# skeskinen/bert.cpp

Measured on AMD Instinct MI355X. Metric: sentences/sec (seq_len=128), higher is better.
Workload: dtype f16; 1 GPU; all-MiniLM-L6-v2 f16, batch=256 seq_len=128; per_gpu_batch=256, global_batch=256, seq_len=128, weights=f16, parallelism=dp1 (replicated weights, sharded sentences)

## Files before the change

bert.cpp_amd/csrc/device.h:

```cpp
#pragma once
#include "kernels.h"

#include <cstdio>
#include <type_traits>
#include <utility>

namespace bert_hip {

typedef _Float16 f16x2 __attribute__((ext_vector_type(2)));
typedef _Float16 f16x4 __attribute__((ext_vector_type(4)));
typedef _Float16 f16x8 __attribute__((ext_vector_type(8)));
typedef float f32x2 __attribute__((ext_vector_type(2)));
typedef float f32x4 __attribute__((ext_vector_type(4)));
typedef float f32x8 __attribute__((ext_vector_type(8)));
typedef float f32x16 __attribute__((ext_vector_type(16)));
typedef uint32_t u32x4 __attribute__((ext_vector_type(4)));
typedef uint32_t u32x16 __attribute__((ext_vector_type(16)));
typedef int32_t i32x4 __attribute__((ext_vector_type(4)));
typedef int32_t i32x16 __attribute__((ext_vector_type(16)));

template <int... I, class F>
__device__ __forceinline__ void static_for_impl(std::integer_sequence<int, I...>, F &&f) {
    (f(std::integral_constant<int, I>{}), ...);
}
// ... 26 lines not shown
    }                                                                                                         \
} while (0)
#define TL_DUMP_RAW(cond, nstamps) do {                                                                      \
    static int tl_shots = 0;                                                                                  \
    if ((cond) && tl_shots++ == 20) {                                                                         \
        (void)hipDeviceSynchronize();                                                                         \
        static unsigned long long tl_h[1024 * 256];                                                           \
        (void)hipMemcpyFromSymbol(tl_h, HIP_SYMBOL(g_timeline), sizeof(tl_h));                                \
        for (int b : {0, 100}) {                                                                              \
            fprintf(stderr, "rawtimeline wg %3d:", b);                                                        \
            for (int i = 0; i < (nstamps); ++i)                                                               \
                fprintf(stderr, " %lld", tl_h[b * 256 + i] ? (long long)(tl_h[b * 256 + i] - tl_h[b * 256]) : -1LL); \
            fprintf(stderr, "\n");                                                                            \
        }                                                                                                     \
    }                                                                                                         \
} while (0)
#else
#define TL_DUMP_RAW(cond, nstamps) do { } while (0)
#define TL_REALTIME_AT(sel, i) do { } while (0)
#define TL_STAMP(i) do { } while (0)
#define TL_STAMP_AT(sel, i) do { } while (0)
#define TL_DUMP(cond, nstamps) do { } while (0)
#endif

__device__ __forceinline__ unsigned lds_addr(const void *p) {
    return (unsigned)(size_t)(__attribute__((address_space(3))) const char *)p;
}
template <bool MEMORY, int OFF, class V = f16x8>
__device__ __forceinline__ V lds_read_b128(unsigned addr) {
    static_assert(sizeof(V) == 16, "ds_read_b128 reads 16 bytes");
    static_assert(OFF >= 0 && OFF < 65536, "ds offset field is 16 bits");
    V v;
    if constexpr (MEMORY) asm volatile("ds_read_b128 %0, %1 offset:%2" : "=v"(v) : "v"(addr), "n"(OFF) : "memory");
    else asm volatile("ds_read_b128 %0, %1 offset:%2" : "=v"(v) : "v"(addr), "n"(OFF));
    return v;
}
template <class V>
__device__ __forceinline__ void landed(V &v) { asm volatile("" : "+v"(v)); }
template <int VM>
__device__ __forceinline__ void dma_barrier() {
    asm volatile("s_waitcnt vmcnt(%0) lgkmcnt(0)\n\ts_barrier" : : "n"(VM) : "memory");
}

__device__ __forceinline__ int off64(int row, int chunk) { return row * 128 + ((chunk ^ ((row >> 1) & 7)) << 4); }

__device__ __forceinline__ float rounded_f32(float v) {
    asm("" : "+v"(v));
    return v;
}

__device__ __forceinline__ void xor32_pair(float &a, float &b) {
    asm("s_nop 1\n\tv_permlane32_swap_b32 %0, %1\n\ts_nop 1" : "+v"(a), "+v"(b));
}
__device__ __forceinline__ float xor32_sum(float v) { float a = v, b = v; xor32_pair(a, b); return a + b; }
__device__ __forceinline__ float xor32_max(float v) { float a = v, b = v; xor32_pair(a, b); return __builtin_fmaxf(a, b); }
__device__ __forceinline__ float wave_sum_f32(float v) {
    v = xor32_sum(v);
    v += __builtin_bit_cast(float, __builtin_amdgcn_ds_swizzle(__builtin_bit_cast(int, v), (16 << 10) | 0x1F));
    v += __builtin_bit_cast(float, __builtin_amdgcn_ds_swizzle(__builtin_bit_cast(int, v), (8 << 10) | 0x1F));
    v += __builtin_bit_cast(float, __builtin_amdgcn_ds_swizzle(__builtin_bit_cast(int, v), (4 << 10) | 0x1F));
    v += __builtin_bit_cast(float, __builtin_amdgcn_mov_dpp(__builtin_bit_cast(int, v), 0x4E, 0xF, 0xF, true));
    v += __builtin_bit_cast(float, __builtin_amdgcn_mov_dpp(__builtin_bit_cast(int, v), 0xB1, 0xF, 0xF, true));
    return v;
}

#ifndef BERT_HIP_EXP16
#define BERT_HIP_EXP16 0
#endif
#if BERT_HIP_EXP16
typedef u32x4 sm_arg_t;
typedef u32x4 sm_exp_t;
__device__ __forceinline__ sm_arg_t softmax_args4(float s0, float s1, float s2, float s3, float s4, float s5, float s6, float s7, float sc, float m) {
    uint32_t a0, a1, a2, a3;
    asm("v_fma_mixlo_f16 %0, %4, %12, -%13\n\t"
        "v_fma_mixlo_f16 %1, %6, %12, -%13\n\t"
        "v_fma_mixlo_f16 %2, %8, %12, -%13\n\t"
        "v_fma_mixlo_f16 %3, %10, %12, -%13\n\t"
        "v_fma_mixhi_f16 %0, %5, %12, -%13\n\t"
        "v_fma_mixhi_f16 %1, %7, %12, -%13\n\t"
        "v_fma_mixhi_f16 %2, %9, %12, -%13\n\t"
        "v_fma_mixhi_f16 %3, %11, %12, -%13"
        : "=&v"(a0), "=&v"(a1), "=&v"(a2), "=&v"(a3)
        : "v"(s0), "v"(s1), "v"(s2), "v"(s3), "v"(s4), "v"(s5), "v"(s6), "v"(s7), "s"(sc), "v"(m));
    return u32x4{a0, a1, a2, a3};
}
__device__ __forceinline__ sm_exp_t softmax_exp4(sm_arg_t a) {
    uint32_t p0, p1, p2, p3;
    asm("v_exp_f16_e32 %0, %4\n\t"
        "v_exp_f16_e32 %1, %5\n\t"
        "v_exp_f16_e32 %2, %6\n\t"
        "v_exp_f16_e32 %3, %7\n\t"
        "v_exp_f16_sdwa %0, %4 dst_sel:WORD_1 dst_unused:UNUSED_PRESERVE src0_sel:WORD_1\n\t"
        "v_exp_f16_sdwa %1, %5 dst_sel:WORD_1 dst_unused:UNUSED_PRESERVE src0_sel:WORD_1\n\t"
        "v_exp_f16_sdwa %2, %6 dst_sel:WORD_1 dst_unused:UNUSED_PRESERVE src0_sel:WORD_1\n\t"
        "v_exp_f16_sdwa %3, %7 dst_sel:WORD_1 dst_unused:UNUSED_PRESERVE src0_sel:WORD_1\n\t"
        "s_nop 0"
        : "=&v"(p0), "=&v"(p1), "=&v"(p2), "=&v"(p3)
        : "v"(a[0]), "v"(a[1]), "v"(a[2]), "v"(a[3]));
    return u32x4{p0, p1, p2, p3};
}
__device__ __forceinline__ void softmax_sum4(sm_exp_t p, float &psum) {
    const f16x2 one = {(_Float16)1.0f, (_Float16)1.0f};
#pragma unroll
    for (int e = 0; e < 4; ++e) {
        const uint32_t pe = p[e];
        psum = __builtin_amdgcn_fdot2(__builtin_bit_cast(f16x2, pe), one, psum, false);
// ... 194 lines not shown
```

bert.cpp_amd/csrc/layer_tail.hip:

```cpp
#include "device.h"

namespace bert_hip {

namespace {

constexpr int LT_TILE = 16384;
#ifndef LT_ABLATE
#define LT_ABLATE 0
#endif
#ifndef LT_UPRIO
#define LT_UPRIO 1
#endif
#ifndef LT_GELU_BATCH
#define LT_GELU_BATCH 0
#endif
#ifndef LT_DMA_SPLIT
#define LT_DMA_SPLIT 1
#endif
#ifndef LT_DPRIO
#define LT_DPRIO 0
#endif

#ifdef BERT_HIP_TIMELINE
static __device__ unsigned long long g_tl_tail[256 * 512];
// ... 5 lines not shown
#endif
#else
#define LT_STAMP_FINE(sel, i) do { } while (0)
#define LT_STAMP(sel, i) do { } while (0)
#endif

struct TailArgs {
    const half_t *ctx, *x;
    const half_t *wo;
    const half_t *w1p;
    const half_t *w2p;
    const uint4 *wo_qs, *w1_qs, *w2_qs;
    const void *wo_sc, *w1_sc, *w2_sc;
    const float *bo, *g1, *be1, *b1, *b2, *g2, *be2;
    half_t *out;
    int I;
};

template <int N>
__device__ __forceinline__ void wait_frags(f16x8 (&f)[4]) {
    asm volatile("s_waitcnt lgkmcnt(%4)" : "+v"(f[0]), "+v"(f[1]), "+v"(f[2]), "+v"(f[3]) : "n"(N) : "memory");
}
template <int N>
__device__ __forceinline__ void wait_lgkm() {
    asm volatile("s_waitcnt lgkmcnt(%0)" : : "n"(N) : "memory");
}
template <int VM>
__device__ __forceinline__ void close_interval(f16x8 (&f)[4]) {
    asm volatile("s_waitcnt vmcnt(%4) lgkmcnt(0)\n\ts_barrier" : "+v"(f[0]), "+v"(f[1]), "+v"(f[2]), "+v"(f[3]) : "n"(VM) : "memory");
}
template <int OFF>
__device__ __forceinline__ f16x8 frag_read(unsigned addr) {
    if (LT_ABLATE & 4) { f16x8 z = (f16x8)(_Float16)0.f; asm volatile("" : "+v"(z) : "v"(addr)); return z; }
    return lds_read_b128<true, OFF>(addr);
}

__device__ __forceinline__ void dma_m0(unsigned lds) {
    if (LT_ABLATE & 1) return;
    asm volatile("s_mov_b32 m0, %0" : : "s"(lds) : "memory");
}
template <int PIECE>
__device__ __forceinline__ void dma_piece(const char *gbase, unsigned voff) {
    if (LT_ABLATE & 1) return;
    asm volatile("global_load_lds_dwordx4 %0, %1 offset:%2" : : "v"(voff), "s"(gbase - PIECE * 1024), "n"(PIECE * 1024) : "memory");
}

__device__ __forceinline__ f32x16 mfma16(const f16x8 &a, const f16x8 &b, const f32x16 &c) {
    if (LT_ABLATE & 8) { f32x16 r = c; asm volatile("" : "+v"(r[0]) : "v"(a), "v"(b)); return r; }
    return __builtin_amdgcn_mfma_f32_32x32x16_f16(a, b, c, 0, 0, 0);
}

}

template <int NT, int WT, bool RAGGED = false>
__device__ __forceinline__ void layer_tail_body(const TailArgs &a, char *smem, const int tok0, const int rows, const int tid) {
    constexpr bool Q4 = WT != GW_F16;
    constexpr int VMQ = Q4 ? 63 : 0;
    constexpr int H = 128 * NT, NBH = 2 * NT, NB = 4 * NT, NQ = 8 * NT, NYH = 4 * NT;
    constexpr int P = NT * NT;
    constexpr int NG = NT;
    constexpr int LAGT = NT + NG;
    const int I = a.I, NC = I / 64;
    const int lane = tid & 63;
    const int wave = __builtin_amdgcn_readfirstlane(tid >> 6);
    const int t = wave & 3, role = wave >> 2;
    const int l31 = lane & 31, hi = lane >> 5;
    const int tok_w = tok0 + t * 32;
    const int row_l = RAGGED ? tok0 + min(t * 32 + l31, rows - 1) : tok_w + l31;

    char *ringU = smem;
    char *ringD = smem + 3 * LT_TILE;
    char *G = smem + 6 * LT_TILE;
    float *ST = (float *)(G + 32768);
    float *cbo = ST + 8 * 64;
    float *cg1 = cbo + H, *cbe1 = cg1 + H, *cb2 = cbe1 + H, *cg2 = cb2 + H, *cbe2 = cg2 + H, *cb1 = cbe2 + H;

    {
        constexpr int NPB = 4;
        const float *const src[6] = {a.bo, a.g1, a.be1, a.b2, a.g2, a.be2};
        float pv[6];
        f32x4 bq[NPB];
#pragma unroll
        for (int k = 0; k < 6; ++k) pv[k] = tid < H ? src[k][tid] : 0.f;
#pragma unroll
        for (int k = 0; k < NPB; ++k) {
            const int i4 = (k * 512 + tid) * 4;
            bq[k] = i4 < I ? *(const f32x4 *)(a.b1 + i4) : f32x4{0.f, 0.f, 0.f, 0.f};
        }
        if (tid < H) {
#pragma unroll
            for (int k = 0; k < 6; ++k) cbo[k * H + tid] = pv[k];
        }
#pragma unroll
        for (int k = 0; k < NPB; ++k) {
            const int i4 = (k * 512 + tid) * 4;
            if (i4 < I + 128) *(f32x4 *)(cb1 + i4) = bq[k];
        }
    }
    f32x16 accp[NBH];
    f16x4 xv[NBH][4];
    {
        const half_t *xr = a.x + (size_t)row_l * H + role * 64 + 4 * hi;
#pragma unroll
        for (int b = 0; b < NBH; ++b)
#pragma unroll
            for (int gq = 0; gq < 4; ++gq) xv[b][gq] = *(const f16x4 *)(xr + (b >> 1) * 128 + (b & 1) * 32 + 8 * gq);
    }
    f16x8 bf[NQ];
// ... 356 lines not shown
                wait_frags<4>(Fb);
                LT_STAMP_FINE(fine, fb0 + 5);
                mm(Fb, I1{});
                LT_STAMP_FINE(fine, fb0 + 6);
                rd(3, Fc);
                wait_frags<4>(Fa);
                LT_STAMP_FINE(fine, fb0 + 7);
                mm(Fa, I2{});
                LT_STAMP_FINE(fine, fb0 + 8);
            } else {
                wait_lgkm<0>();
                bias_landed();
                static_for<12>([&](auto s_tag) __attribute__((always_inline)) { fill(std::integral_constant<int, 4 + decltype(s_tag)::value>{}); });
            }
            static_assert(MAXF <= 2, "two GELU batches per interval at most");
            pre_close();
            if constexpr (MMA) close_interval<VMQ>(Fc); else dma_barrier<VMQ>();
            next_slot();
        };
        using TT = std::true_type; using FF = std::false_type;
        LT_STAMP(tlU, 393);
        __builtin_amdgcn_s_setprio(LT_UPRIO);
        auto u_chunk = [&](auto par_tag, auto first_tag, int c) __attribute__((always_inline)) {
            constexpr bool FIRST = decltype(first_tag)::value;
            static_for<NT>([&](auto j_tag) __attribute__((always_inline)) {
                constexpr int j = decltype(j_tag)::value;
                constexpr bool carry = !(FIRST && j == 0), gelu = !FIRST && j < NG;
                u_interval(par_tag, j_tag, TT{}, std::integral_constant<bool, gelu>{}, std::integral_constant<bool, carry>{}, c);
            });
        };
        u_chunk(std::integral_constant<int, 0>{}, TT{}, 0);
        for (int c = 1; c + 1 < NC; c += 2) {
            u_chunk(std::integral_constant<int, 1>{}, FF{}, c);
            u_chunk(std::integral_constant<int, 0>{}, FF{}, c + 1);
        }
        u_chunk(std::integral_constant<int, 1>{}, FF{}, NC - 1);
        static_for<LAGT>([&](auto k_tag) __attribute__((always_inline)) {
            constexpr int k = decltype(k_tag)::value;
            if constexpr (k < NG)
                u_interval(std::integral_constant<int, 0>{}, std::integral_constant<int, k>{}, FF{}, TT{}, std::integral_constant<bool, k == 0>{}, NC);
            else {
                if constexpr (k == NG) {
                    char *const xu = ringU + t * (NYH * 1024) + lane * 16;
#pragma unroll
                    for (int m = 0; m < NYH; ++m) *(f16x8 *)(xu + m * 1024) = Y[8 * (m >> 2) + (m & 3)];
                }
                pre_close(); dma_barrier<VMQ>(); next_slot();
            }
        });
        static_assert(LAGT > NG, "U needs an idle interval to hand its half of y over");
        asm volatile("s_barrier" ::: "memory");
        asm volatile("s_barrier" ::: "memory");
        store_rows();
        return;
    } else {
        f16x8 yh[NYH];
        static_for<NBH>([&](auto b_tag) __attribute__((always_inline)) {
            constexpr int b = decltype(b_tag)::value;
            normalise_block(b_tag, yh[2 * b], yh[2 * b + 1]);
            *(f16x8 *)(xch + (2 * b) * 1024) = yh[2 * b];
            *(f16x8 *)(xch + (2 * b + 1) * 1024) = yh[2 * b + 1];
        });
        LT_STAMP(tlD, 400);
        asm volatile("s_waitcnt lgkmcnt(0)\n\ts_barrier" ::: "memory");
        f32x16 acc2[NB];
        static_for<NBH>([&](auto b_tag) __attribute__((always_inline)) {
            constexpr int b = decltype(b_tag)::value, n3 = b >> 1, obp = b & 1;
            f32x4 bu[4], bd[4];
#pragma unroll
            for (int gq = 0; gq < 4; ++gq) {
                bu[gq] = *(const f32x4 *)(cb2 + n3 * 128 + obp * 32 + 8 * gq + 4 * hi);
                bd[gq] = *(const f32x4 *)(cb2 + n3 * 128 + 64 + obp * 32 + 8 * gq + 4 * hi);
            }
#pragma unroll
            for (int gq = 0; gq < 4; ++gq)
#pragma unroll
                for (int e = 0; e < 4; ++e) {
                    acc2[4 * n3 + obp][4 * gq + e] = bu[gq][e];
                    acc2[4 * n3 + 2 + obp][4 * gq + e] = (float)yh[2 * b + (gq >> 1)][4 * (gq & 1) + e] + bd[gq][e];
                }
            asm volatile("" ::: "memory");
        });
        __builtin_amdgcn_s_waitcnt(0xc07f);
        const unsigned aD = aR + 3 * LT_TILE;
        const unsigned offI = rows_offset(I);
        auto dma_down = [&](int c, int n3, unsigned tile) __attribute__((always_inline)) {
            if constexpr (Q4) q4_request_rows(a.w2_qs, a.w2_sc, n3 * (I / 64) + c);
            else dma128(w2p + (size_t)n3 * 128 * I + c * 64, offI, I * 2, tile);
        };
        const unsigned aG = lds_addr(G) + (unsigned)(t * 8192 + lane * 16);
        const unsigned offU = up_offset();
        const int NUP = NC * NT;
        auto request = [&](auto up_tag, auto down_tag, int iu, int id) __attribute__((always_inline)) {
            const int s2 = slot_plus2();
            if constexpr (decltype(up_tag)::value) dma_up(iu / NT, iu % NT, offU, ldsU + s2 * LT_TILE);
            if constexpr (decltype(down_tag)::value) dma_down(id / NT, id % NT, ldsD + s2 * LT_TILE);
        };
        using TT = std::true_type; using FF = std::false_type;
        if (LT_DPRIO) __builtin_amdgcn_s_setprio(LT_DPRIO);
        static_for<LAGT>([&](auto k_tag) __attribute__((always_inline)) {
            constexpr int k = decltype(k_tag)::value;
            constexpr bool dn = k >= LAGT - 2;
            if constexpr (k >= 1) q4_expand_up(ringU + slot_plus1() * LT_TILE);
            if constexpr (k == LAGT - 1) q4_expand_rows(PERMUTED{}, ringD + slot_plus1() * LT_TILE);
            request(TT{}, std::integral_constant<bool, dn>{}, k + 2, k - (LAGT - 2));
            pre_close();
// ... 57 lines not shown
            });
        };
        static_assert(LAGT == 2 * NT, "the request schedule below assumes D runs two chunks behind");
        (void)NUP;
        for (int c = 0; c + 3 < NC; ++c) d_chunk(std::integral_constant<int, NT>{}, FF{}, TT{}, c);
        d_chunk(std::integral_constant<int, NT - 2>{}, FF{}, TT{}, NC - 3);
        d_chunk(std::integral_constant<int, 0>{}, FF{}, FF{}, NC - 2);
        d_chunk(std::integral_constant<int, 0>{}, TT{}, FF{}, NC - 1);

        {
            char *S = smem + t * (64 * H);
            int lane = (int)__builtin_amdgcn_mbcnt_hi(~0u, __builtin_amdgcn_mbcnt_lo(~0u, 0u));
            asm volatile("" : "+v"(lane));
            const int hi = lane >> 5;
            {
                const char *const xu = ringU + t * (NYH * 1024) + lane * 16;
#pragma unroll
                for (int n3 = 0; n3 < NT; ++n3) {
                    f16x8 yu[4];
#pragma unroll
                    for (int m = 0; m < 4; ++m) yu[m] = *(const f16x8 *)(xu + (4 * n3 + m) * 1024);
#pragma unroll
                    for (int m = 0; m < 4; ++m)
#pragma unroll
                        for (int e = 0; e < 8; ++e) acc2[4 * n3 + (m >> 1)][8 * (m & 1) + e] += (float)yu[m][e];
                    asm volatile("" ::: "memory");
                }
            }
            asm volatile("s_waitcnt lgkmcnt(0)\n\ts_barrier" ::: "memory");
            float s1 = 0.f, s2 = 0.f;
#pragma unroll
            for (int n = 0; n < NB; ++n)
#pragma unroll
                for (int r = 0; r < 16; ++r) { s1 += acc2[n][r]; s2 = __builtin_fmaf(acc2[n][r], acc2[n][r], s2); }
            s1 += __shfl_xor(s1, 32);
            s2 += __shfl_xor(s2, 32);
            float rstd, nmr;
            layernorm_scale(s1, s2, 1.0f / H, rstd, nmr);
#pragma unroll
            for (int n = 0; n < NB; ++n) {
                f32x4 gv[4], bv[4];
#pragma unroll
                for (int g4 = 0; g4 < 4; ++g4) { gv[g4] = *(const f32x4 *)(cg2 + 32 * n + 8 * g4 + 4 * hi); bv[g4] = *(const f32x4 *)(cbe2 + 32 * n + 8 * g4 + 4 * hi); }
#pragma unroll
                for (int s = 0; s < 2; ++s) {
                    const int q = 2 * n + s;
                    f16x8 o;
#pragma unroll
                    for (int hq = 0; hq < 2; ++hq)
#pragma unroll
                        for (int e = 0; e < 4; ++e)
                            o[4 * hq + e] = (_Float16)rounded_f32(__builtin_fmaf(acc2[n][8 * s + 4 * hq + e], gv[2 * s + hq][e] * rstd, __builtin_fmaf(gv[2 * s + hq][e], nmr, bv[2 * s + hq][e])));
                    *(f16x8 *)(S + q * 1024 + ((lane + 2 * q) & 63) * 16) = o;
                }
                asm volatile("" ::: "memory");
            }
            LT_STAMP(tlD, 401);
            asm volatile("s_waitcnt lgkmcnt(0)\n\ts_barrier" ::: "memory");
        }
        store_rows();
    }
}

template <int NT, int WT>
__global__ __launch_bounds__(512) void layer_tail_kernel(TailArgs a) {
    extern __shared__ __attribute__((aligned(16))) char smem[];
    layer_tail_body<NT, WT>(a, smem, (int)blockIdx.x * 128, 128, (int)threadIdx.x);
}

static size_t layer_tail_lds(int H, int I) {
    return (size_t)6 * LT_TILE + 32768 + 8 * 64 * 4 + (size_t)(6 * H + I + 128) * sizeof(float);
}

#ifndef BERT_HIP_PHASES_ONLY

bool layer_tail_supported(const GemmWeight &Wo, const GemmWeight &W1, const GemmWeight &W2) {
    const int H = W1.K, I = W1.N;
    if (Wo.type != W1.type || W1.type != W2.type) return false;
    if (W1.type == GW_F16 ? (!Wo.w16 || !W1.w16p || !W2.w16p) : (!Wo.qs || !W1.qs || !W2.qs)) return false;
    if (Wo.N != H || Wo.K != H || W2.N != H || W2.K != I) return false;
    if (H % 128 != 0 || H < 256 || H > 384 || I % 128 != 0 || I < 256) return false;
    return layer_tail_lds(H, I) <= 160 * 1024;
}

void launch_layer_tail(const GemmWeight &Wo, const GemmWeight &W1, const GemmWeight &W2, const half_t *ctx, const half_t *x,
                        const float *bo, const float *g1, const float *be1, const float *b1, const float *b2,
                        const float *g2, const float *be2, half_t *out, int M_pad, hipStream_t stream) {
    TailArgs a;
    a.ctx = ctx; a.x = x; a.wo = Wo.w16; a.w1p = W1.w16p; a.w2p = W2.w16p;
    a.wo_qs = Wo.qs; a.w1_qs = W1.qs; a.w2_qs = W2.qs; a.wo_sc = Wo.sc; a.w1_sc = W1.sc; a.w2_sc = W2.sc;
    a.bo = bo; a.g1 = g1; a.be1 = be1; a.b1 = b1; a.b2 = b2; a.g2 = g2; a.be2 = be2; a.out = out;
    a.I = W1.N;
    const int H = W1.K;
    const size_t lds = layer_tail_lds(H, a.I);
    static DeviceFlags configured[6];
    auto go = [&](auto kernel, int which) {
        configure_once(configured[which], [&] { (void)hipFuncSetAttribute((const void *)kernel, hipFuncAttributeMaxDynamicSharedMemorySize, 160 * 1024); });
        BERT_LAUNCH(kernel, dim3(M_pad / 128), dim3(512), lds, stream, a);
#ifdef BERT_HIP_TIMELINE
        static int shots = 0;
        if (M_pad >= 128 * 256 && shots++ == 20) {
            (void)hipDeviceSynchronize();
            static unsigned long long h[256 * 512];
            (void)hipMemcpyFromSymbol(h, HIP_SYMBOL(g_tl_tail), sizeof(h));
            for (int b : {0, 100}) {
                const unsigned long long *r = h + b * 512, t0 = r[0];
                auto rel = [&](int i) { return r[i] ? (long long)(r[i] - t0) : -1LL; };
                fprintf(stderr, "tail wg %d phases:", b);
                for (int i = 384; i < 402; ++i) fprintf(stderr, " %d:%lld", i, rel(i));
                fprintf(stderr, "\nt3 wg %d inside U's intervals 40..45 (start, reads issued, carried done, g0 landed, g0 done, g1 landed, g1 done, g2 landed, g2 done):", b);
                for (int k = 0; k < 6; ++k) {
                    fprintf(stderr, " [");
                    for (int i = 1; i < 9; ++i) fprintf(stderr, "%lld ", r[402 + k * 10 + i] ? (long long)(r[402 + k * 10 + i] - r[402 + k * 10]) : -1LL);
                    fprintf(stderr, "]");
// ... 21 lines not shown
```

bert.cpp_amd/csrc/model_kernel.hip:

```cpp
#define BERT_HIP_PHASES_ONLY
#include "qkv_attention2.hip"
#include "layer_tail.hip"
#undef BERT_HIP_PHASES_ONLY
#include "pool_normalize.h"

namespace bert_hip {

#ifdef BERT_HIP_MODEL_TIMELINE
static __device__ unsigned long long g_tl_model[1024 * 32];
#define MK_STAMP(i) do { const int mk_i = (i); if (threadIdx.x == 0 && mk_i < 32) g_tl_model[(blockIdx.x & 1023) * 32 + mk_i] = __builtin_amdgcn_s_memrealtime(); } while (0)
#else
#define MK_STAMP(i) do { } while (0)
#endif

namespace {

constexpr int MODEL_MAX_LAYERS = 12;

struct ModelLayerArgs {
    const half_t *wqkv, *wo, *w1p, *w2p;
    const float *bqkv, *bo, *g1, *be1, *b1, *b2, *g2, *be2;
};
struct ModelArgs {
    half_t *x, *ctx;
    const int32_t *cu;
    const int2 *groups;
    const int *n_groups;
    int n_layer, n_head, n_sent, I, slot_mask;
    float *pooled;
    int *status;
    int max_len;
    ModelLayerArgs layer[MODEL_MAX_LAYERS];
};

}

template <int NT, bool RAGGED>
__global__ __launch_bounds__(512, 2) void model_kernel(ModelArgs m) {
    extern __shared__ __attribute__((aligned(16))) char smem[];
    const int window = (int)blockIdx.x;
    int tok0 = window * 128, rows = 128, first = window, count = 1;
    if constexpr (RAGGED) {
        if (m.groups) {
            if (m.n_groups && window >= *m.n_groups) return;
            const int2 g = m.groups[window];
            first = g.x; count = g.y;
        }
        if (count <= 0 || first >= m.n_sent) return;
        tok0 = m.cu[first];
        rows = min(m.cu[first + count] - tok0, 128);
    }
    const int wave_index = __builtin_amdgcn_readfirstlane((int)threadIdx.x >> 6);
    auto thread_id = [&]() __attribute__((always_inline)) {
        int ln = (int)__builtin_amdgcn_mbcnt_hi(~0u, __builtin_amdgcn_mbcnt_lo(~0u, 0u)), w = wave_index;
        asm volatile("" : "+v"(ln), "+s"(w));
        return w * 64 + ln;
    };
    MK_STAMP(0);
    const int n_layer = rows > 0 ? m.n_layer : 0;
    for (int l = 0; l < n_layer; ++l) {
        const ModelLayerArgs &L = m.layer[l];
        int tid = thread_id();
        {
            Qkv2Args q;
            q.x = m.x; q.w = L.wqkv; q.qs = nullptr; q.sc = nullptr; q.bias = L.bqkv; q.cu = m.cu; q.groups = RAGGED ? m.groups : nullptr; q.n_groups = nullptr;
            q.out = m.ctx; q.n_head = m.n_head; q.n_sent = m.n_sent; q.spw = 1; q.slot_mask = m.slot_mask;
            qkv_attention2_body<2 * NT, NT, GW_F16>(q, smem, window, tid);
        }
        __builtin_amdgcn_fence(__ATOMIC_RELEASE, "workgroup");
        asm volatile("s_waitcnt vmcnt(0) lgkmcnt(0)\n\ts_barrier" ::: "memory");
        __builtin_amdgcn_fence(__ATOMIC_ACQUIRE, "workgroup");
        MK_STAMP(1 + 2 * l);
        tid = thread_id();
        {
            TailArgs t;
            t.ctx = m.ctx; t.x = m.x; t.wo = L.wo; t.w1p = L.w1p; t.w2p = L.w2p;
            t.wo_qs = t.w1_qs = t.w2_qs = nullptr; t.wo_sc = t.w1_sc = t.w2_sc = nullptr;
            t.bo = L.bo; t.g1 = L.g1; t.be1 = L.be1; t.b1 = L.b1; t.b2 = L.b2; t.g2 = L.g2; t.be2 = L.be2; t.out = m.x; t.I = m.I;
            layer_tail_body<NT, GW_F16, RAGGED>(t, smem, tok0, rows, tid);
        }
        __builtin_amdgcn_fence(__ATOMIC_RELEASE, "workgroup");
        asm volatile("s_waitcnt vmcnt(0) lgkmcnt(0)\n\ts_barrier" ::: "memory");
        __builtin_amdgcn_fence(__ATOMIC_ACQUIRE, "workgroup");
        MK_STAMP(2 + 2 * l);
    }
    if (m.pooled) {
        const int tid = thread_id();
        for (int j = 0; j < count; ++j) {
            const int b = first + j, t0 = m.cu[b];
            int n = m.cu[b + 1] - t0;
            if (!RAGGED && (t0 != tok0 || n != 128)) n = -1;
            pool_normalize_sentence(m.x, t0, n, b, 128 * NT, m.max_len, m.status, m.pooled, (float *)smem, tid, tid < 256);
            __syncthreads();
        }
    }
    MK_STAMP(1 + 2 * n_layer);
}

bool model_kernel_supported(const GemmWeight &Wqkv, const GemmWeight &Wo, const GemmWeight &W1, const GemmWeight &W2, int n_layer,
                            int n_head, int d_head, int max_len) {
    const int H = n_head * d_head;
    return n_layer <= MODEL_MAX_LAYERS && (H == 256 || H == 384) && max_len >= 1 && max_len <= 128 &&
           Wqkv.type == GW_F16 && Wo.type == GW_F16 && qkv_attention2_supported(Wqkv, n_head, d_head, max_len) && layer_tail_supported(Wo, W1, W2);
}

void launch_model_kernel(const ModelLayerWeights *layers, int n_layer, half_t *x, half_t *ctx, const int32_t *cu_seqlens, int n_sentences,
                         int n_tokens, const int2 *groups, int n_groups, const int *n_groups_dev, int n_head, float *pooled, int max_len,
                         int *status, int slots, hipStream_t stream) {
    ModelArgs m;
    m.pooled = pooled; m.status = status; m.max_len = max_len;
    m.x = x; m.ctx = ctx; m.cu = cu_seqlens; m.groups = groups; m.n_groups = n_groups_dev;
    m.n_layer = n_layer; m.n_head = n_head; m.n_sent = n_sentences; m.I = layers[0].W1->N; m.slot_mask = slots - 1;
    for (int l = 0; l < n_layer; ++l) {
        const ModelLayerWeights &s = layers[l];
        ModelLayerArgs &d = m.layer[l];
        d.wqkv = s.Wqkv->w16; d.wo = s.Wo->w16; d.w1p = s.W1->w16p; d.w2p = s.W2->w16p;
        d.bqkv = s.bqkv; d.bo = s.bo; d.g1 = s.g1; d.be1 = s.be1; d.b1 = s.b1; d.b2 = s.b2; d.g2 = s.g2; d.be2 = s.be2;
    }
    const int H = layers[0].W1->K, KT = H / 64, GB = KT / 2;
    const size_t lds_q = (size_t)3 * GB * Q2_TILE + 2 * (2 * Q2_WIN * 64 + 32 * Q2_VT_LD * 2) + (size_t)2 * H * sizeof(float);
    const size_t lds = std::max(lds_q, layer_tail_lds(H, m.I));
    const bool full = (long long)n_sentences * 128 == n_tokens;
    const int grid = full || !groups ? n_sentences : n_groups;
    static DeviceFlags configured[4];
    auto go = [&](auto kernel, int which) {
        configure_once(configured[which], [&] { (void)hipFuncSetAttribute((const void *)kernel, hipFuncAttributeMaxDynamicSharedMemorySize, 160 * 1024); });
        BERT_LAUNCH(kernel, dim3(grid), dim3(512), lds, stream, m);
#ifdef BERT_HIP_MODEL_TIMELINE
        static int shots = 0;
        if (grid >= 256 && shots++ == 30) {
            (void)hipDeviceSynchronize();
            static unsigned long long h[1024 * 32];
            (void)hipMemcpyFromSymbol(h, HIP_SYMBOL(g_tl_model), sizeof(h));
            const int nw = grid < 1024 ? grid : 1024, ns = 2 + 2 * n_layer;
            unsigned long long t0 = ~0ull;
            for (int w = 0; w < nw; ++w) t0 = h[w * 32] < t0 ? h[w * 32] : t0;
            fprintf(stderr, "model_kernel timeline, %d workgroups (us after the first workgroup's start: min mean max):\n", nw);
// ... 35 lines not shown
```

bert.cpp_amd/csrc/qkv_attention2.hip:

```cpp
#include "device.h"

#ifndef Q2_PM
#define Q2_PM 3
#endif
#ifndef Q2_PRIO
#define Q2_PRIO 0
#endif

namespace bert_hip {

namespace {

constexpr int Q2_WIN = 128;
constexpr int Q2_TILE = 12288;
constexpr int Q2_VT_LD = Q2_WIN + 4;

struct Qkv2Args {
    const half_t *x;
    const half_t *w;
    const uint4 *qs;
    const void *sc;
    const float *bias;
    const int32_t *cu;
    const int2 *groups;
    const int *n_groups;
    half_t *out;
    int n_head, n_sent, spw;
    int slot_mask;
};

__device__ __forceinline__ int q2_off32(int row, int chunk) { return row * 64 + ((chunk ^ ((row >> 2) & 3)) << 4); }

__device__ __forceinline__ void q2_wait6(f16x8 (&f)[2][3]) {
    asm volatile("s_waitcnt lgkmcnt(6)"
                 : "+v"(f[0][0]), "+v"(f[0][1]), "+v"(f[0][2]), "+v"(f[1][0]), "+v"(f[1][1]), "+v"(f[1][2]) : : "memory");
}
template <int VM>
__device__ __forceinline__ void q2_slab_barrier(f16x8 (&f)[2][3]) {
    asm volatile("s_waitcnt vmcnt(%6) lgkmcnt(0)\n\ts_barrier"
                 : "+v"(f[0][0]), "+v"(f[0][1]), "+v"(f[0][2]), "+v"(f[1][0]), "+v"(f[1][1]), "+v"(f[1][2]) : "n"(VM) : "memory");
}
__device__ __forceinline__ void q2_wait14(f16x8 (&f)[2][3]) {
    asm volatile("s_waitcnt lgkmcnt(14)"
                 : "+v"(f[0][0]), "+v"(f[0][1]), "+v"(f[0][2]), "+v"(f[1][0]), "+v"(f[1][1]), "+v"(f[1][2]) : : "memory");
}
__device__ __forceinline__ void q2_wait0_bias(f16x8 (&f)[2][3], f32x4 (&bq)[4], f32x4 (&bk)[4]) {
    asm volatile("s_waitcnt lgkmcnt(0)"
                 : "+v"(f[0][0]), "+v"(f[0][1]), "+v"(f[0][2]), "+v"(f[1][0]), "+v"(f[1][1]), "+v"(f[1][2]),
                   "+v"(bq[0]), "+v"(bq[1]), "+v"(bq[2]), "+v"(bq[3]), "+v"(bk[0]), "+v"(bk[1]), "+v"(bk[2]), "+v"(bk[3]) : : "memory");
}

}

template <int KT, int GB, int WT>
__device__ __forceinline__ void qkv_attention2_body(const Qkv2Args &a, char *smem, const int window, const int tid) {
    constexpr bool Q4 = WT != GW_F16;
    constexpr int H = 64 * KT, NBAR = KT / GB, SLAB = GB * Q2_TILE, PPS = 3 * GB;
    static_assert(KT == 2 * GB && NBAR == 2, "");
    constexpr int QKV_BYTES = 2 * Q2_WIN * 64 + 32 * Q2_VT_LD * 2;
    char *RING = smem;
    char *QKV = smem + 3 * SLAB;
    float *BS = (float *)(QKV + 2 * QKV_BYTES);

    const int lane = tid & 63;
    const int wave = __builtin_amdgcn_readfirstlane(tid >> 6);
    const int l31 = lane & 31, hi = lane >> 5;
    const int blk = wave & 3;
    const int n_head = a.n_head;
    TL_STAMP_AT(tid == 256, 120);
    TL_REALTIME_AT(tid == 256, 121);
    TL_STAMP_AT(tid == 0, 250);
    TL_REALTIME_AT(tid == 0, 251);

    const int wp = blk;
    const unsigned loff = (unsigned)(((wp * 8 + (lane >> 3)) * H + (((lane & 7) ^ (((wp & 1) << 2) | ((lane >> 4) & 3))) * 8)) * 2);
    auto dma_piece = [&](const char *hbase, auto j_tag, int dslot, auto i_tag) __attribute__((always_inline)) {
        constexpr int i = decltype(i_tag)::value, j = decltype(j_tag)::value, t = i / 3, rb = i % 3;
        const char *src = hbase + ((size_t)rb * H * H + (size_t)(j * GB + t) * 64) * 2;
        __builtin_amdgcn_global_load_lds(AS_GLOBAL(src + loff), AS_LDS(RING + dslot * SLAB + t * Q2_TILE + rb * 4096 + wp * 1024), 16, 0, 0);
    };
    const char *const wbase = (const char *)a.w;
    if constexpr (!Q4) {
        if (wave >= 4) static_for<PPS>([&](auto i) __attribute__((always_inline)) { dma_piece(wbase, std::integral_constant<int, 0>{}, 0, i); });
    }

    int first, count;
    if (a.groups) {
        if (a.n_groups && window >= *a.n_groups) {
            asm volatile("s_waitcnt vmcnt(0)" ::: "memory");
            return;
        }
        const int2 g = a.groups[window];
        first = g.x; count = g.y;
    }
    else { first = window * a.spw; count = min(a.spw, a.n_sent - first); }
    if (count <= 0) {
        asm volatile("s_waitcnt vmcnt(0)" ::: "memory");
        return;
    }
    const int slot = blk * 32 + l31;
    int gtok = -1, k0 = 0, k1 = 0;
    {
        const int place = a.groups ? 128 : 128 / a.spw;
        int off = 0;
        for (int j = 0; j < count; ++j) {
            const int t0 = a.cu[first + j], n = min(a.cu[first + j + 1] - t0, place);
            if (slot >= off && slot < off + n) { gtok = t0 + slot - off; k0 = off; k1 = off + n; }
            off = (off + n + a.slot_mask) & ~a.slot_mask;
        }
    }

    if (wave >= 4) {
        f16x8 bf[4 * KT];
        {
            const int gt = gtok >= 0 ? gtok : a.cu[first];
            const half_t *xr = a.x + (size_t)gt * H + 8 * hi;
#pragma unroll
            for (int ks = 0; ks < 4 * KT; ++ks) asm volatile("global_load_dwordx4 %0, %1, off" : "=v"(bf[ks]) : "v"(xr + 16 * ks));
        }
        if constexpr (!Q4) static_for<PPS>([&](auto i) __attribute__((always_inline)) { dma_piece(wbase, std::integral_constant<int, NBAR - 1>{}, 1, i); });

        constexpr int NRAW = GB;
        [[maybe_unused]] RawBlock raw[NRAW];
        auto q4_image_of_lane = [&]() __attribute__((always_inline)) {
            int ln = (int)__builtin_amdgcn_mbcnt_hi(~0u, __builtin_amdgcn_mbcnt_lo(~0u, 0u));
            asm volatile("" : "+v"(ln));
            return (ln >> 1) * 128 + (((4 * (ln & 1)) ^ ((ln >> 2) & 7)) << 4);
        };
        auto q4_rb = [&](int hq, int j, int i) __attribute__((always_inline)) { return (blk + i + 2 * hq + j) & 3; };
        auto q4_request = [&](int hq, int j, int i) __attribute__((always_inline)) {
            if constexpr (Q4) {
                const int rb = q4_rb(hq, j, i);
                if (rb == 3) return;
                const int sbase = ((rb * (H / 128) + (hq >> 2)) * (H / 64) + j * GB + i) * 256 + (hq & 3) * 64;
                raw[i] = q4_load_block<WT>(a.qs + sbase, WT == GW_Q4_0 ? (const void *)((const unsigned short *)a.sc + sbase) : (const void *)((const unsigned *)a.sc + sbase), (size_t)lane);
            }
        };
        auto q4_expand = [&](int hq, int j, int dslot, int i) __attribute__((always_inline)) {
            if constexpr (Q4) {
                const int rb = q4_rb(hq, j, i);
                if (rb == 3) return;
                char *const base = RING + dslot * SLAB + i * Q2_TILE + rb * 4096;
                const int q4_image = q4_image_of_lane();
                q4_expand_block<WT, false>(raw[i], [&](int k) __attribute__((always_inline)) { return base + (q4_image ^ (k << 4)); });
            }
        };
        if constexpr (Q4) {
            RawBlock first[2][NRAW];
#pragma unroll
            for (int j = 0; j < 2; ++j)
#pragma unroll
                for (int i = 0; i < NRAW; ++i) {
                    q4_request(0, j, i);
                    first[j][i] = raw[i];
                }
#pragma unroll
            for (int j = 0; j < 2; ++j)
#pragma unroll
                for (int i = 0; i < NRAW; ++i) {
                    raw[i] = first[j][i];
                    q4_expand(0, j, j, i);
                }
        }
        const unsigned aX0 = lds_addr(RING) + off64(l31, hi);
        unsigned aS[4];
        int rslot = 0;
        auto set_slot = [&]() __attribute__((always_inline)) {
#pragma unroll
// ... 182 lines not shown
                    }
                }
                if constexpr (WB) {
                    if (kt == Q2_PM) {
                        if (tb < 8) TL_STAMP_AT(tl_sel, 128 + 6 * tb + 1);
                        asm volatile("s_barrier" ::: "memory");
                        if (tb < 8) TL_STAMP_AT(tl_sel, 128 + 6 * tb + 2);
                    }
                }
            }
            mx = xor32_max(mx) * sc;
            mx = fmaxf(mx, -3.0e38f);
            float psum = 0.f;
            f32x16 o;
#pragma unroll
            for (int r = 0; r < 16; ++r) o[r] = 0.f;
#pragma unroll
            for (int kt = 0; kt < 4; ++kt) {
                if (FAST || (need & (1u << kt))) {
#pragma unroll
                    for (int st = 0; st < 2; ++st) {
                        const f16x8 pf = softmax_p8(s[kt][8 * st], s[kt][8 * st + 1], s[kt][8 * st + 2], s[kt][8 * st + 3], s[kt][8 * st + 4],
                                                    s[kt][8 * st + 5], s[kt][8 * st + 6], s[kt][8 * st + 7], sc, mx, psum);
                        const int key0 = kt * 32 + 16 * st + 4 * hi;
                        const half_t *vr = VT + l31 * Q2_VT_LD + key0;
                        const f16x4 v0 = *(const f16x4 *)vr, v1 = *(const f16x4 *)(vr + 8);
                        f16x8 vf;
#pragma unroll
                        for (int e = 0; e < 4; ++e) { vf[e] = v0[e]; vf[4 + e] = v1[e]; }
                        o = __builtin_amdgcn_mfma_f32_32x32x16_f16(vf, pf, o, 0, 0, 0);
                    }
                }
                if constexpr (WB) {
                    if (kt + 4 == Q2_PM) {
                        if (tb < 8) TL_STAMP_AT(tl_sel, 128 + 6 * tb + 1);
                        asm volatile("s_barrier" ::: "memory");
                        if (tb < 8) TL_STAMP_AT(tl_sel, 128 + 6 * tb + 2);
                    }
                }
            }
            psum = xor32_sum(psum);
            if (gtok >= 0) {
                const float inv = 1.0f / psum;
                half_t *op = a.out + (size_t)gtok * H + hh * 32;
#pragma unroll
                for (int gq = 0; gq < 4; ++gq) {
                    f16x4 ov;
#pragma unroll
                    for (int e = 0; e < 4; ++e) ov[e] = (_Float16)rounded_f32(o[4 * gq + e] * inv);
                    *(f16x4 *)(op + 8 * gq + 4 * hi) = ov;
                }
            }
        };
        const bool fast = need == 0xFu && inner == 0xFu;
        asm volatile("s_barrier" ::: "memory");
        asm volatile("s_barrier" ::: "memory");
        for (int h = 1; h < n_head; ++h) {
            if (h < 8) TL_STAMP_AT(tl_sel, 128 + 6 * h);
            if (fast) attend(h - 1, std::true_type{}, std::true_type{}, h);
            else attend(h - 1, std::true_type{}, std::false_type{}, h);
            if (h < 8) TL_STAMP_AT(tl_sel, 128 + 6 * h + 5);
            asm volatile("s_barrier" ::: "memory");
        }
        TL_STAMP_AT(tl_sel, 190);
        if (fast) attend(n_head - 1, std::false_type{}, std::true_type{}, 0);
        else attend(n_head - 1, std::false_type{}, std::false_type{}, 0);
        TL_STAMP_AT(tl_sel, 192);
        TL_STAMP_AT(tl_sel, 252);
        TL_REALTIME_AT(tl_sel, 253);
    }
}

template <int KT, int GB, int WT>
__global__ __launch_bounds__(512, 2) void qkv_attention2_kernel(Qkv2Args a) {
    extern __shared__ __attribute__((aligned(16))) char smem[];
    qkv_attention2_body<KT, GB, WT>(a, smem, (int)blockIdx.x, (int)threadIdx.x);
}

#ifndef BERT_HIP_PHASES_ONLY
constexpr int BW_THREADS = 512;

template <int SLOT>
__global__ __launch_bounds__(BW_THREADS) void build_windows_kernel(const int32_t *__restrict__ cu, int B, int2 *__restrict__ windows,
                                                                   int *__restrict__ n_windows) {
    constexpr int BW_STATES = 128 / SLOT + 1;
    __shared__ unsigned char exit_state[BW_THREADS][BW_STATES];
    __shared__ int closes[BW_THREADS][BW_STATES];
    __shared__ int opened[BW_THREADS][BW_STATES];
    __shared__ int entry_fill[BW_THREADS], entry_first[BW_THREADS], entry_index[BW_THREADS];
    const int t = threadIdx.x, per = (B + BW_THREADS - 1) / BW_THREADS, n_blocks = per ? (B + per - 1) / per : 0;
    const int b0 = min(B, t * per), b1 = min(B, b0 + per);

    int fill[BW_STATES], n_closed[BW_STATES], first[BW_STATES];
#pragma unroll
    for (int e = 0; e < BW_STATES; ++e) { fill[e] = e * SLOT; n_closed[e] = 0; first[e] = -1; }
    for (int b = b0; b < b1; ++b) {
        const int n = cu[b + 1] - cu[b];
#pragma unroll
        for (int e = 0; e < BW_STATES; ++e) {
            if (fill[e] == 0) first[e] = b;
            else if (fill[e] + n > 128) { ++n_closed[e]; first[e] = b; fill[e] = 0; }
            fill[e] = min(128, (fill[e] + n + SLOT - 1) & ~(SLOT - 1));
        }
    }
#pragma unroll
    for (int e = 0; e < BW_STATES; ++e) {
        exit_state[t][e] = (unsigned char)(fill[e] / SLOT); closes[t][e] = n_closed[e]; opened[t][e] = first[e];
    }
    __syncthreads();
    if (t == 0) {
        int e = 0, open_first = 0, index = 0;
        for (int k = 0; k < n_blocks; ++k) {
            entry_fill[k] = e * SLOT; entry_first[k] = open_first; entry_index[k] = index;
            index += closes[k][e];
            if (opened[k][e] >= 0) open_first = opened[k][e];
            e = exit_state[k][e];
        }
        if (B > 0) windows[index++] = make_int2(open_first, B - open_first);
        *n_windows = index;
// ... 69 lines not shown
```

Measured before the change: 324,400 sentences/s.

## Hand layer output to next layer's QKV in registers for full windows

In the non-ragged persistent model kernel, the layer tail's final LayerNorm output fragments are converted into MFMA operand layout (via permlane32 swaps) and kept in registers. The next layer's QKV/attention phase then reads them directly instead of reloading x from global memory. A FULL specialization also drops the group/window bookkeeping and the slow attention path for full windows. The cost is more live VGPRs across phases, which could cause spills or lower occupancy.

```diff
diff --git a/bert.cpp_amd/csrc/device.h b/bert.cpp_amd/csrc/device.h
--- a/bert.cpp_amd/csrc/device.h
+++ b/bert.cpp_amd/csrc/device.h
@@ -102,6 +102,12 @@
 __device__ __forceinline__ void xor32_pair(float &a, float &b) {
     asm("s_nop 1\n\tv_permlane32_swap_b32 %0, %1\n\ts_nop 1" : "+v"(a), "+v"(b));
 }
+__device__ __forceinline__ f16x8 result_to_operand_fragment(const f16x8 &v) {
+    const u32x4 d = __builtin_bit_cast(u32x4, v);
+    uint32_t d0 = d[0], d1 = d[1], d2 = d[2], d3 = d[3];
+    asm("s_nop 1\n\tv_permlane32_swap_b32 %0, %2\n\tv_permlane32_swap_b32 %1, %3\n\ts_nop 1" : "+v"(d0), "+v"(d1), "+v"(d2), "+v"(d3));
+    return __builtin_bit_cast(f16x8, u32x4{d0, d1, d2, d3});
+}
 __device__ __forceinline__ float xor32_sum(float v) { float a = v, b = v; xor32_pair(a, b); return a + b; }
 __device__ __forceinline__ float xor32_max(float v) { float a = v, b = v; xor32_pair(a, b); return __builtin_fmaxf(a, b); }
 __device__ __forceinline__ float wave_sum_f32(float v) {
diff --git a/bert.cpp_amd/csrc/layer_tail.hip b/bert.cpp_amd/csrc/layer_tail.hip
--- a/bert.cpp_amd/csrc/layer_tail.hip
+++ b/bert.cpp_amd/csrc/layer_tail.hip
@@ -81,8 +81,10 @@
 
 }
 
-template <int NT, int WT, bool RAGGED = false>
-__device__ __forceinline__ void layer_tail_body(const TailArgs &a, char *smem, const int tok0, const int rows, const int tid) {
+template <int NT, int WT, bool RAGGED, bool HANDOVER>
+__device__ __forceinline__ void layer_tail_body(const TailArgs &a, char *smem, const int tok0, const int rows, const int tid,
+                                                [[maybe_unused]] f16x8 (&xnext)[8 * NT]) {
+    static_assert(!(HANDOVER && RAGGED), "a ragged window's rows are packed: its lanes are not the window phase's slots");
     constexpr bool Q4 = WT != GW_F16;
     constexpr int VMQ = Q4 ? 63 : 0;
     constexpr int H = 128 * NT, NBH = 2 * NT, NB = 4 * NT, NQ = 8 * NT, NYH = 4 * NT;
@@ -545,6 +547,10 @@
         asm volatile("s_barrier" ::: "memory");
         asm volatile("s_barrier" ::: "memory");
         store_rows();
+        if constexpr (HANDOVER) {
+#pragma unroll
+            for (int q = 0; q < NQ; ++q) asm volatile("" : "=v"(xnext[q]));
+        }
         return;
     } else {
         f16x8 yh[NYH];
@@ -708,6 +714,7 @@
                         for (int e = 0; e < 4; ++e)
                             o[4 * hq + e] = (_Float16)rounded_f32(__builtin_fmaf(acc2[n][8 * s + 4 * hq + e], gv[2 * s + hq][e] * rstd, __builtin_fmaf(gv[2 * s + hq][e], nmr, bv[2 * s + hq][e])));
                     *(f16x8 *)(S + q * 1024 + ((lane + 2 * q) & 63) * 16) = o;
+                    if constexpr (HANDOVER) xnext[q] = result_to_operand_fragment(o);
                 }
                 asm volatile("" ::: "memory");
             }
@@ -716,6 +723,12 @@
         }
         store_rows();
     }
+}
+
+template <int NT, int WT, bool RAGGED = false>
+__device__ __forceinline__ void layer_tail_body(const TailArgs &a, char *smem, const int tok0, const int rows, const int tid) {
+    f16x8 unused[8 * NT];
+    layer_tail_body<NT, WT, RAGGED, false>(a, smem, tok0, rows, tid, unused);
 }
 
 template <int NT, int WT>
diff --git a/bert.cpp_amd/csrc/model_kernel.hip b/bert.cpp_amd/csrc/model_kernel.hip
--- a/bert.cpp_amd/csrc/model_kernel.hip
+++ b/bert.cpp_amd/csrc/model_kernel.hip
@@ -58,31 +58,47 @@
     };
     MK_STAMP(0);
     const int n_layer = rows > 0 ? m.n_layer : 0;
-    for (int l = 0; l < n_layer; ++l) {
-        const ModelLayerArgs &L = m.layer[l];
-        int tid = thread_id();
-        {
-            Qkv2Args q;
-            q.x = m.x; q.w = L.wqkv; q.qs = nullptr; q.sc = nullptr; q.bias = L.bqkv; q.cu = m.cu; q.groups = RAGGED ? m.groups : nullptr; q.n_groups = nullptr;
-            q.out = m.ctx; q.n_head = m.n_head; q.n_sent = m.n_sent; q.spw = 1; q.slot_mask = m.slot_mask;
-            qkv_attention2_body<2 * NT, NT, GW_F16>(q, smem, window, tid);
-        }
+    auto window_phase = [&](const ModelLayerArgs &L, auto xregs_tag, const f16x8 *xf) __attribute__((always_inline)) {
+        const int tid = thread_id();
+        Qkv2Args q;
+        q.x = m.x; q.w = L.wqkv; q.qs = nullptr; q.sc = nullptr; q.bias = L.bqkv; q.cu = m.cu; q.groups = RAGGED ? m.groups : nullptr; q.n_groups = nullptr;
+        q.out = m.ctx; q.n_head = m.n_head; q.n_sent = m.n_sent; q.spw = 1; q.slot_mask = m.slot_mask;
+        qkv_attention2_body<2 * NT, NT, GW_F16, !RAGGED, decltype(xregs_tag)::value>(q, smem, window, tid, xf);
+    };
+    auto tail_phase = [&](const ModelLayerArgs &L, f16x8 (&xf)[8 * NT]) __attribute__((always_inline)) {
+        const int tid = thread_id();
+        TailArgs t;
+        t.ctx = m.ctx; t.x = m.x; t.wo = L.wo; t.w1p = L.w1p; t.w2p = L.w2p;
+        t.wo_qs = t.w1_qs = t.w2_qs = nullptr; t.wo_sc = t.w1_sc = t.w2_sc = nullptr;
+        t.bo = L.bo; t.g1 = L.g1; t.be1 = L.be1; t.b1 = L.b1; t.b2 = L.b2; t.g2 = L.g2; t.be2 = L.be2; t.out = m.x; t.I = m.I;
+        layer_tail_body<NT, GW_F16, RAGGED, !RAGGED>(t, smem, tok0, rows, tid, xf);
+    };
+    auto hand_over = [&]() __attribute__((always_inline)) {
         __builtin_amdgcn_fence(__ATOMIC_RELEASE, "workgroup");
         asm volatile("s_waitcnt vmcnt(0) lgkmcnt(0)\n\ts_barrier" ::: "memory");
         __builtin_amdgcn_fence(__ATOMIC_ACQUIRE, "workgroup");
-        MK_STAMP(1 + 2 * l);
-        tid = thread_id();
-        {
-            TailArgs t;
-            t.ctx = m.ctx; t.x = m.x; t.wo = L.wo; t.w1p = L.w1p; t.w2p = L.w2p;
-            t.wo_qs = t.w1_qs = t.w2_qs = nullptr; t.wo_sc = t.w1_sc = t.w2_sc = nullptr;
-            t.bo = L.bo; t.g1 = L.g1; t.be1 = L.be1; t.b1 = L.b1; t.b2 = L.b2; t.g2 = L.g2; t.be2 = L.be2; t.out = m.x; t.I = m.I;
-            layer_tail_body<NT, GW_F16, RAGGED>(t, smem, tok0, rows, tid);
+    };
+    if constexpr (RAGGED) {
+        for (int l = 0; l < n_layer; ++l) {
+            f16x8 none[8 * NT];
+            window_phase(m.layer[l], std::false_type{}, nullptr);
+            hand_over();
+            MK_STAMP(1 + 2 * l);
+            tail_phase(m.layer[l], none);
+            hand_over();
+            MK_STAMP(2 + 2 * l);
         }
-        __builtin_amdgcn_fence(__ATOMIC_RELEASE, "workgroup");
-        asm volatile("s_waitcnt vmcnt(0) lgkmcnt(0)\n\ts_barrier" ::: "memory");
-        __builtin_amdgcn_fence(__ATOMIC_ACQUIRE, "workgroup");
-        MK_STAMP(2 + 2 * l);
+    } else {
+        if (n_layer > 0) window_phase(m.layer[0], std::false_type{}, nullptr);
+        for (int l = 0; l < n_layer; ++l) {
+            hand_over();
+            MK_STAMP(1 + 2 * l);
+            f16x8 xf[8 * NT];
+            tail_phase(m.layer[l], xf);
+            hand_over();
+            MK_STAMP(2 + 2 * l);
+            if (l + 1 < n_layer) window_phase(m.layer[l + 1], std::true_type{}, xf);
+        }
     }
     if (m.pooled) {
         const int tid = thread_id();
diff --git a/bert.cpp_amd/csrc/qkv_attention2.hip b/bert.cpp_amd/csrc/qkv_attention2.hip
--- a/bert.cpp_amd/csrc/qkv_attention2.hip
+++ b/bert.cpp_amd/csrc/qkv_attention2.hip
@@ -52,8 +52,10 @@
 
 }
 
-template <int KT, int GB, int WT>
-__device__ __forceinline__ void qkv_attention2_body(const Qkv2Args &a, char *smem, const int window, const int tid) {
+template <int KT, int GB, int WT, bool FULL = false, bool XREGS = false>
+__device__ __forceinline__ void qkv_attention2_body(const Qkv2Args &a, char *smem, const int window, const int tid,
+                                                    [[maybe_unused]] const f16x8 *xf = nullptr) {
+    static_assert(FULL || !XREGS, "fragments handed over in registers: full windows only");
     constexpr bool Q4 = WT != GW_F16;
     constexpr int H = 64 * KT, NBAR = KT / GB, SLAB = GB * Q2_TILE, PPS = 3 * GB;
     static_assert(KT == 2 * GB && NBAR == 2, "");
@@ -85,22 +87,26 @@
     }
 
     int first, count;
-    if (a.groups) {
-        if (a.n_groups && window >= *a.n_groups) {
+    if constexpr (FULL) { first = window; count = 1; }
+    else {
+        if (a.groups) {
+            if (a.n_groups && window >= *a.n_groups) {
+                asm volatile("s_waitcnt vmcnt(0)" ::: "memory");
+                return;
+            }
+            const int2 g = a.groups[window];
+            first = g.x; count = g.y;
+        }
+        else { first = window * a.spw; count = min(a.spw, a.n_sent - first); }
+        if (count <= 0) {
             asm volatile("s_waitcnt vmcnt(0)" ::: "memory");
             return;
         }
-        const int2 g = a.groups[window];
-        first = g.x; count = g.y;
-    }
-    else { first = window * a.spw; count = min(a.spw, a.n_sent - first); }
-    if (count <= 0) {
-        asm volatile("s_waitcnt vmcnt(0)" ::: "memory");
-        return;
     }
     const int slot = blk * 32 + l31;
     int gtok = -1, k0 = 0, k1 = 0;
-    {
+    if constexpr (FULL) { gtok = window * Q2_WIN + slot; k1 = Q2_WIN; }
+    else {
         const int place = a.groups ? 128 : 128 / a.spw;
         int off = 0;
         for (int j = 0; j < count; ++j) {
@@ -112,8 +118,11 @@
 
     if (wave >= 4) {
         f16x8 bf[4 * KT];
-        {
-            const int gt = gtok >= 0 ? gtok : a.cu[first];
+        if constexpr (XREGS) {
+#pragma unroll
+            for (int ks = 0; ks < 4 * KT; ++ks) bf[ks] = xf[ks];
+        } else {
+            const int gt = FULL || gtok >= 0 ? gtok : a.cu[first];
             const half_t *xr = a.x + (size_t)gt * H + 8 * hi;
 #pragma unroll
             for (int ks = 0; ks < 4 * KT; ++ks) asm volatile("global_load_dwordx4 %0, %1, off" : "=v"(bf[ks]) : "v"(xr + 16 * ks));
@@ -402,19 +411,19 @@
                 }
             }
         };
-        const bool fast = need == 0xFu && inner == 0xFu;
+        const bool fast = FULL || (need == 0xFu && inner == 0xFu);
         asm volatile("s_barrier" ::: "memory");
         asm volatile("s_barrier" ::: "memory");
         for (int h = 1; h < n_head; ++h) {
             if (h < 8) TL_STAMP_AT(tl_sel, 128 + 6 * h);
-            if (fast) attend(h - 1, std::true_type{}, std::true_type{}, h);
-            else attend(h - 1, std::true_type{}, std::false_type{}, h);
+            if (FULL || fast) attend(h - 1, std::true_type{}, std::true_type{}, h);
+            else if constexpr (!FULL) attend(h - 1, std::true_type{}, std::false_type{}, h);
             if (h < 8) TL_STAMP_AT(tl_sel, 128 + 6 * h + 5);
             asm volatile("s_barrier" ::: "memory");
         }
         TL_STAMP_AT(tl_sel, 190);
-        if (fast) attend(n_head - 1, std::false_type{}, std::true_type{}, 0);
-        else attend(n_head - 1, std::false_type{}, std::false_type{}, 0);
+        if (FULL || fast) attend(n_head - 1, std::false_type{}, std::true_type{}, 0);
+        else if constexpr (!FULL) attend(n_head - 1, std::false_type{}, std::false_type{}, 0);
         TL_STAMP_AT(tl_sel, 192);
         TL_STAMP_AT(tl_sel, 252);
         TL_REALTIME_AT(tl_sel, 253);
```

After: 329,300 sentences/s, median of 6. 1.02x the previous value.
